# nii-yamagishilab/NELE-GAN

Measured on AMD Instinct MI355X. Metric: utterances/sec per GAN_epoch step (G+D+metric loss), higher is better.
Workload: dtype bf16

## Files before the change

### nele_gan_amd/csrc/haspi.hip

```cpp
#include "common.h"
#include "ws_arena.h"
#include <type_traits>
#include <cstdlib>

#define HP_NCH 32
#define HP_FS 24000.0
#define HP_LEVEL 65.0
#define HP_NBASIS 6
#define HP_NMOD 10
#define HP_NWIN 32769
#define HP_NTAB 512
#define HP_SPACE 9
#define HP_NFILT 52
#define HP_NHALF 26

typedef float hp_env_t;

struct HaspiWs {
    double* win;
    float* r24;
    double* mid;
    hp_env_t* ctl;
    hp_env_t* env;
    double* bw;
// ... 477 lines not shown
    if (loss < thrOHC) { attnOHC = 0.8 * loss; attnIHC = 0.2 * loss; }
    else { attnOHC = 0.8 * thrOHC; attnIHC = 0.2 * thrOHC + (loss - thrOHC); }
    const double r = attnOHC / 50.0;
    const double BW = 1.0 + r + 2.0 * (r * r * r * r * r * r);
    const double lowknee = attnOHC + 30.0, upamp = 30.0 + 70.0 / CR0;
    const double CR = (100.0 - lowknee) / (upamp + attnOHC - lowknee);
    double* p = ws.loss + (size_t)sig * 5 * HP_NCH + ch;
    p[0] = attnOHC; p[HP_NCH] = BW; p[2 * HP_NCH] = lowknee; p[3 * HP_NCH] = CR; p[4 * HP_NCH] = attnIHC;
}

__device__ __forceinline__ void hp_rotate(double& cold, double& sold, double cn, double sn);
__device__ __forceinline__ double hp_gammatone_wave(const double* __restrict__ xin, int n24, const GtCoef c, double cf, int part,
                                                    hp_env_t* __restrict__ out) {
    const double tpt = 2.0 * M_PI / HP_FS;
    const double cn = cos(tpt * cf), sn = sin(tpt * cf);
    double cold = 1.0, sold = 0.0;
    double r0 = 0, r1 = 0, r2 = 0, r3 = 0;
    double ss = 0.0;
    for (int n0 = 0; n0 < n24; n0 += HP_CH) {
        double xc[HP_CH];
#pragma unroll
        for (int u = 0; u < HP_CH; ++u) xc[u] = xin[n0 + u];
        double eo[HP_CH];
#pragma unroll
        for (int u = 0; u < HP_CH; ++u) {
            if (n0 + u > 0) hp_rotate(cold, sold, cn, sn);
            const double xr = xc[u] * (part ? sold : cold);
            const double yr = xr + r0;
            r0 = c.a1 * xr + c.a1 * yr + r1;
            r1 = c.a5 * xr + c.a2 * yr + r2;
            r2 = c.a3 * yr + r3;
            r3 = c.a4 * yr;
            const double yo = lane_xor32(yr);
            const double e2 = yr * yr + yo * yo;
            eo[u] = e2;
            ss += (n0 + u < n24) ? e2 : 0.0;
        }
        if (part == 0) {
#pragma unroll
            for (int u = 0; u < HP_CH; ++u) out[(size_t)(n0 + u) * HP_NCH] = (hp_env_t)eo[u];
        }
    }
    return ss;
}

#define GS_RC 16
#define GS_LC 1536
#define GS_MAXC 160
__device__ __forceinline__ void hp_rotate(double& cold, double& sold, double cn, double sn) {
    const double arg = fma(sold, sn, cold * cn);
    sold = fma(sold, cn, -(cold * sn));
    cold = arg;
}
__device__ __forceinline__ void hp_gt_step(const GtCoef& c, double x, double y, double& r0, double& r1, double& r2, double& r3) {
    r0 = fma(c.a1, x + y, r1);
    r1 = fma(c.a5, x, fma(c.a2, y, r2));
    r2 = fma(c.a3, y, r3);
    r3 = c.a4 * y;
}
__global__ __launch_bounds__(128) void haspi_pmat_kernel(HaspiWs ws, int lc, int signal, int sig0, int nsig) {
    const int ch = threadIdx.x & 31, k = threadIdx.x >> 5;
    const int row = signal ? hp_row(blockIdx.x, sig0, nsig) : 0;
    const double BW = signal ? ws.bw[(size_t)row * HP_NCH + ch] : hp_bw1(ch);
    const GtCoef c = hp_gt(BW, hp_cfreq(ch));
    double r0 = (k == 0), r1 = (k == 1), r2 = (k == 2), r3 = (k == 3);
    for (int n = 0; n < lc; ++n) {
        const double yr = r0;
        r0 = c.a1 * yr + r1;
        r1 = c.a2 * yr + r2;
        r2 = c.a3 * yr + r3;
        r3 = c.a4 * yr;
    }
    double* P = ws.pmat + ((size_t)(signal ? 1 + row : 0) * HP_NCH + ch) * 16;
    P[0 * 4 + k] = r0; P[1 * 4 + k] = r1; P[2 * 4 + k] = r2; P[3 * 4 + k] = r3;
}

template <bool SIGNAL>
__global__ __launch_bounds__(64) void haspi_bank_prefix_kernel(HaspiWs ws, int sig0, int nsig) {
    const int row = hp_row(blockIdx.x, sig0, nsig), lane = threadIdx.x, ch = lane & 31;
    const int n24 = hp_n24(ws, row >> 1);
    const int nch = ((n24 + GS_RC - 1) / GS_RC * GS_RC + ws.lc - 1) / ws.lc;
    const double* P = ws.pmat + ((size_t)(SIGNAL ? 1 + row : 0) * HP_NCH + ch) * 16;
    double Pm[16];
#pragma unroll
    for (int q = 0; q < 16; ++q) Pm[q] = P[q];
    double* est = ws.est + (size_t)row * ws.nchunk * 256 + lane;
    double r0 = 0, r1 = 0, r2 = 0, r3 = 0;
    constexpr int G = 8;
    for (int j0 = 0; j0 < nch; j0 += G) {
        double e[G][4];
#pragma unroll
        for (int g = 0; g < G; ++g) {
            const int j = min(j0 + g, nch - 1);
#pragma unroll
            for (int q = 0; q < 4; ++q) e[g][q] = est[(size_t)j * 256 + 64 * q];
        }
#pragma unroll
        for (int g = 0; g < G; ++g) {
            if (j0 + g < nch) {
                double* o = est + (size_t)(j0 + g) * 256;
                o[0] = r0; o[64] = r1; o[128] = r2; o[192] = r3;
                const double t0 = ((Pm[0] * r0 + Pm[1] * r1) + (Pm[2] * r2 + Pm[3] * r3)) + e[g][0];
                const double t1 = ((Pm[4] * r0 + Pm[5] * r1) + (Pm[6] * r2 + Pm[7] * r3)) + e[g][1];
                const double t2 = ((Pm[8] * r0 + Pm[9] * r1) + (Pm[10] * r2 + Pm[11] * r3)) + e[g][2];
                const double t3 = ((Pm[12] * r0 + Pm[13] * r1) + (Pm[14] * r2 + Pm[15] * r3)) + e[g][3];
                r0 = t0; r1 = t1; r2 = t2; r3 = t3;
            }
        }
    }
}

#define GL_N 2048
#define GL_W 256
#define GL_U 8
__device__ __forceinline__ float hp_log2f(float x) { return __builtin_amdgcn_logf(x); }
__device__ __forceinline__ float hp_exp2f(float x) { return __builtin_amdgcn_exp2f(x); }
struct IhcC { double R2, R12C1, R23C2, a11, a12, a21, a22, denom, R1inv, c10, c11, c12, c20, c21, c22; };
__device__ __forceinline__ IhcC hp_ihc_consts() {
    const double delta = 2.0;
    const double tau1 = 0.001 * 2, tau2 = 0.001 * 60;
    const double T = 1 / HP_FS;
    const double R1 = 1 / delta, R2 = 0.5 * (1 - R1), R3 = R2;
    const double C1 = tau1 * (R1 + R2) / (R1 * R2);
    const double C2 = tau2 / ((R1 + R2) * R3);
    IhcC k;
    k.a11 = R1 + R2 + R1 * R2 * (C1 / T); k.a12 = -R1; k.a21 = -R3; k.a22 = R2 + R3 + R2 * R3 * (C2 / T);
    k.denom = 1.0 / (k.a11 * k.a22 - k.a21 * k.a12);
    k.R1inv = 1.0 / R1; k.R12C1 = R1 * R2 * (C1 / T); k.R23C2 = R2 * R3 * (C2 / T); k.R2 = R2;
    k.c10 = k.denom * k.a22 * k.R2;  k.c11 = k.denom * k.a22 * k.R12C1;  k.c12 = -k.denom * k.a12 * k.R23C2;
    k.c20 = -k.denom * k.a21 * k.R2; k.c21 = -k.denom * k.a21 * k.R12C1; k.c22 = k.denom * k.a11 * k.R23C2;
    return k;
}
__device__ __forceinline__ void hp_ihc_step(const IhcC& k, double V0, double& V1, double& V2) {
    const double t1 = fma(k.c12, V2, fma(k.c11, V1, V0 * k.c10));
    const double t2 = fma(k.c22, V2, fma(k.c21, V1, V0 * k.c20));
    V1 = t1; V2 = t2;
}

template <bool SIGNAL, bool PASS2, bool BM = false, bool GAIN = false>
__global__ __launch_bounds__(64) void haspi_bank_scan_kernel(HaspiWs ws, int sig0) {
    const int b = blockIdx.z, sig = sig0 + blockIdx.y, lane = threadIdx.x, ch = lane & 31;
    const int chunk = 2 * blockIdx.x + (lane >> 5);
    const int row = 2 * b + sig, lc = ws.lc;
    const int n24 = hp_n24(ws, b);
    const int n0 = chunk * lc, n1 = min(n0 + lc, (n24 + GS_RC - 1) / GS_RC * GS_RC);
    if (n0 >= n1) return;
    const double cf = hp_cfreq(ch);
    const GtCoef c = hp_gt(SIGNAL ? ws.bw[(size_t)row * HP_NCH + ch] : hp_bw1(ch), cf);
    const double tpt = 2.0 * M_PI / HP_FS;
    const double cn = cos(tpt * cf), sn = sin(tpt * cf);
    double* est = ws.est + ((size_t)row * ws.nchunk + chunk) * 256 + ch;
    double r0 = 0, r1 = 0, r2 = 0, r3 = 0, i0 = 0, i1 = 0, i2 = 0, i3 = 0;
    if (PASS2) {
        r0 = est[0]; r1 = est[64]; r2 = est[128]; r3 = est[192];
        i0 = est[32]; i1 = est[96]; i2 = est[160]; i3 = est[224];
    }
    double cold, sold;
    {
        const double ang = tpt * cf * (double)(n0 - 1);
        cold = cos(ang);
        sold = -sin(ang);
    }
    const double* xin = ws.mid + (size_t)row * ws.n24p;
    hp_env_t* out = (SIGNAL ? ws.env : ws.ctl) + ((size_t)row * ws.n24p) * HP_NCH + ch;
    float* cph = BM ? ws.cphi + ((size_t)row * ws.n24p) * HP_NCH + ch : nullptr;
    double ss = 0.0;
    const hp_env_t* ctl = ws.ctl + (size_t)row * ws.n24p * HP_NCH + ch;
    const float TEN_LOG10_2 = 3.0102999566398120f, LOG2_10_OVER_20 = 0.16609640474436813f;
    float slope = 0.f, c_off = 0.f, s_off = 0.f;
    double gz = 0.0, V1 = 0.0, V2 = 0.0;
    const double gb0 = 0.095107983402496, ga1 = -0.809784033195007;
    const IhcC ik = hp_ihc_consts();
    float knee = 30.0f, attn = 0.f;
    if (GAIN) {
        const HpLoss ls = hp_loss(ws, sig, ch);
        slope = (float)(1.0 - (1.0 / ls.CR));
        knee = (float)ls.lowknee; attn = (float)ls.attnOHC;
        c_off = (float)(HP_LEVEL + 20.0 * log10(hp_gt(hp_bw1(ch), cf).gain));
        s_off = (float)(HP_LEVEL - ls.attnIHC + 20.0 * log10(c.gain));
        for (int n = max(0, n0 - GL_W); n < n0; n += GL_U) {
            float gc[GL_U];
#pragma unroll
            for (int u = 0; u < GL_U; ++u) gc[u] = ctl[(size_t)(n + u) * HP_NCH];
#pragma unroll
            for (int u = 0; u < GL_U; ++u) {
                float le = c_off + TEN_LOG10_2 * hp_log2f(gc[u]);
                le = fminf(fmaxf(le, knee), 100.0f);
                const double gx = (double)hp_exp2f((-attn - (le - knee) * slope) * LOG2_10_OVER_20);
                const double y = gb0 * gx + gz;
                gz = gb0 * gx - ga1 * y;
            }
        }
    }
    for (int nb = n0; nb < n1; nb += GS_RC) {
        double xc[GS_RC];
        const hp_env_t* ctl_nb = ctl + (size_t)nb * HP_NCH;
        hp_env_t* out_nb = out + (size_t)nb * HP_NCH;
        float* cph_nb = BM ? cph + (size_t)nb * HP_NCH : nullptr;
#pragma unroll
        for (int u = 0; u < GS_RC / 2; ++u) {
            const double2 v = *reinterpret_cast<const double2*>(xin + nb + 2 * u);
            xc[2 * u] = v.x; xc[2 * u + 1] = v.y;
        }
        float eo[GS_RC], co[BM ? GS_RC : 1];
        auto bank = [&](auto tail_tag) {
            constexpr bool TAIL = decltype(tail_tag)::value;
#pragma unroll
            for (int u = 0; u < GS_RC; ++u) {
                hp_rotate(cold, sold, cn, sn);
                const double xr = xc[u] * cold, xi = xc[u] * sold;
                const double yr = xr + r0, yi = xi + i0;
                hp_gt_step(c, xr, yr, r0, r1, r2, r3);
                hp_gt_step(c, xi, yi, i0, i1, i2, i3);
                if (PASS2) {
                    const double e2 = yr * yr + yi * yi;
                    eo[u] = (float)e2;
                    if (!SIGNAL || BM) ss += (!TAIL || nb + u < n24) ? e2 : 0.0;
                    if (BM) co[u] = e2 > 0.0 ? (float)((yr * cold + yi * sold) / sqrt(e2)) : 0.f;
                }
            }
        };
        if (PASS2 && (!SIGNAL || BM) && nb + GS_RC > n24) bank(std::true_type{}); else bank(std::false_type{});
        if (GAIN) {
            float gc[GS_RC];
#pragma unroll
            for (int u = 0; u < GS_RC; ++u) gc[u] = ctl_nb[u * HP_NCH];
#pragma unroll
            for (int u = 0; u < GS_RC; ++u) {
                float le = c_off + TEN_LOG10_2 * hp_log2f(gc[u]);
                le = fminf(fmaxf(le, knee), 100.0f);
                const double gx = (double)hp_exp2f((-attn - (le - knee) * slope) * LOG2_10_OVER_20);
                const double yl = gb0 * gx + gz;
                gz = gb0 * gx - ga1 * yl;
                const float g = (float)yl;
                float y = s_off + TEN_LOG10_2 * hp_log2f(g * g * eo[u]);
                y = y > 0.0f ? y : 0.0f;
                eo[u] = y;
                hp_ihc_step(ik, (double)y, V1, V2);
            }
        }
        if (PASS2) {
#pragma unroll
            for (int u = 0; u < GS_RC; ++u) out_nb[u * HP_NCH] = eo[u];
            if (BM) {
#pragma unroll
                for (int u = 0; u < GS_RC; ++u) cph_nb[u * HP_NCH] = co[u];
            }
        }
    }
    if (!PASS2) {
        est[0] = r0; est[64] = r1; est[128] = r2; est[192] = r3;
        est[32] = i0; est[96] = i1; est[160] = i2; est[224] = i3;
    } else if (!SIGNAL) {
        ws.ssp[((size_t)row * ws.nchunk + chunk) * HP_NCH + ch] = ss;
    } else if (BM) {
        ws.sse[((size_t)row * ws.nchunk + chunk) * HP_NCH + ch] = ss;
    }
    if (GAIN) {
        const int ncg = (ws.n24p + ws.lcg - 1) / ws.lcg;
        double* ihe = ws.ihe + ((size_t)row * ncg + chunk) * 64 + ch;
        ihe[0] = V1; ihe[32] = V2;
    }
}

template <bool SIGNAL>
__global__ __launch_bounds__(512) void haspi_bank_tail_kernel(HaspiWs ws, int sig0, int nsig, int full, int nrows) {
    __shared__ double stage[2][64][GS_RC + 1];
    __shared__ int wred[8];
    const int id = (int)blockIdx.x, slot = id >> 3, cgrp = slot & 3, rest = slot >> 2;
    const int ncg = (ws.nchunk + 63) / 64;
    const int ridx = (rest / ncg) * 8 + (id & 7);
    if (ridx >= nrows) return;
    const int row = hp_row(ridx, sig0, nsig), b = row >> 1;
    const int tid = threadIdx.x, lane = tid & 63, wv = tid >> 6, ch = 8 * cgrp + wv;
    const int c0 = 64 * (rest % ncg), chunk = c0 + lane, lc = ws.lc;
    const int n24 = hp_n24(ws, b), nend = (n24 + GS_RC - 1) / GS_RC * GS_RC;
    const int n0 = chunk * lc, n1 = min(n0 + lc, nend);
    const bool live = n0 < n1;
    const double cf = hp_cfreq(ch);
    const double BW = SIGNAL ? ws.bw[(size_t)row * HP_NCH + ch] : hp_bw1(ch);
    const GtCoef c = hp_gt(BW, cf);
    const double tpt = 2.0 * M_PI / HP_FS;
    int W;
    {
        const double la = BW * tpt * (24.7 + cf / 9.26449) * 1.019;
        const double npk = fmax(3.0 / la, 1.0);
        const double peak = 3.0 * log(npk) - la * npk;
        double nn = 60.0 / la;
        for (int it = 0; it < 6; ++it) nn = (50.66 - peak + 3.0 * log(nn)) / la;
        W = ((int)nn + 1 + GS_RC) / GS_RC * GS_RC;
        W = min(W, lc);
        if (full == 1) W = lc;
        if (full == 2) W = GS_RC;
    }
    if (lane == 0) wred[wv] = W;
    __syncthreads();
    int Wmax = wred[0];
#pragma unroll
    for (int q = 1; q < 8; ++q) Wmax = max(Wmax, wred[q]);
    const double cn = cos(tpt * cf), sn = sin(tpt * cf);
    double cold, sold;
    {
        const double ang = tpt * cf * (double)(n1 - W - 1);
        cold = cos(ang);
        sold = -sin(ang);
    }
    const double* xin = ws.mid + (size_t)row * ws.n24p;
    const int cc = tid >> 3, part = tid & 7;
    const int cn0 = (c0 + cc) * lc, cn1 = min(cn0 + lc, nend);
    const double* psrc = xin + (cn1 - Wmax + 2 * part);
    const int pfirst = (cn0 < cn1) ? cn0 - (cn1 - Wmax + 2 * part) : 0x7fffffff;
    double2 pv = (0 >= pfirst) ? *reinterpret_cast<const double2*>(psrc) : make_double2(0.0, 0.0);
    double r0 = 0, r1 = 0, r2 = 0, r3 = 0, i0 = 0, i1 = 0, i2 = 0, i3 = 0;
    const int tjoin = Wmax - W;
    for (int t = 0, it = 0; t < Wmax; t += GS_RC, ++it) {
        double (*st)[GS_RC + 1] = stage[it & 1];
        st[cc][2 * part] = pv.x; st[cc][2 * part + 1] = pv.y;
        __syncthreads();
        if (t + GS_RC < Wmax) pv = (t + GS_RC >= pfirst) ? *reinterpret_cast<const double2*>(psrc + t + GS_RC) : make_double2(0.0, 0.0);
        if (t >= tjoin) {
            double xc[GS_RC];
#pragma unroll
            for (int u = 0; u < GS_RC; ++u) xc[u] = st[lane][u];
#pragma unroll
            for (int u = 0; u < GS_RC; ++u) {
                hp_rotate(cold, sold, cn, sn);
                const double xr = xc[u] * cold, xi = xc[u] * sold;
                const double yr = xr + r0, yi = xi + i0;
                hp_gt_step(c, xr, yr, r0, r1, r2, r3);
                hp_gt_step(c, xi, yi, i0, i1, i2, i3);
            }
        }
    }
    if (live) {
        double* est = ws.est + ((size_t)row * ws.nchunk + chunk) * 256 + ch;
        est[0] = r0; est[64] = r1; est[128] = r2; est[192] = r3;
        est[32] = i0; est[96] = i1; est[160] = i2; est[224] = i3;
    }
}
__global__ void haspi_bw_kernel(HaspiWs ws, int sig0, int nsig) {
    const int row = hp_row(blockIdx.x, sig0, nsig), ch = threadIdx.x;
    const double bw1 = hp_bw1(ch);
    const GtCoef cc = hp_gt(bw1, hp_cfreq(ch));
    const int n24 = hp_n24(ws, row >> 1);
    const int nch = (n24 + ws.lc - 1) / ws.lc;
    double ss = 0.0;
    for (int c = 0; c < nch; ++c) ss += ws.ssp[((size_t)row * ws.nchunk + c) * HP_NCH + ch];
    ss *= cc.gain * cc.gain;
    const double cdB = 20.0 * log10(sqrt(ss / (double)n24)) + HP_LEVEL;
    const double bwmin = hp_loss(ws, row & 1, ch).BWmin;
    double BW;
    if (cdB < 50.0) BW = bwmin;
    else if (cdB > 100.0) BW = bw1;
    else BW = bwmin + ((cdB - 50.0) / 50.0) * (bw1 - bwmin);
    ws.bw[(size_t)row * HP_NCH + ch] = BW;
}

#ifdef NELE_AB
__global__ __launch_bounds__(64) void haspi_control_kernel(HaspiWs ws, int sig0) {
    const int b = blockIdx.y, sig = sig0 + blockIdx.x, lane = threadIdx.x, part = lane >> 5, ch = lane & 31;
    const double cf = hp_cfreq(ch), bw1 = hp_bw1(ch);
    const double* xin = ws.mid + ((size_t)b * 2 + sig) * ws.n24p;
    hp_env_t* out = ws.ctl + (((size_t)b * 2 + sig) * ws.n24p) * HP_NCH + ch;
    const GtCoef cc = hp_gt(bw1, cf);
    const int n24 = hp_n24(ws, b);
    const double ss = (cc.gain * cc.gain) * hp_gammatone_wave(xin, n24, cc, cf, part, out);
    if (part == 0) {
        const double cdB = 20.0 * log10(sqrt(ss / (double)n24)) + HP_LEVEL;
        const double bwmin = hp_loss(ws, sig, ch).BWmin;
        double BW;
        if (cdB < 50.0) BW = bwmin;
        else if (cdB > 100.0) BW = bw1;
        else BW = bwmin + ((cdB - 50.0) / 50.0) * (bw1 - bwmin);
        ws.bw[((size_t)b * 2 + sig) * HP_NCH + ch] = BW;
    }
}
#endif

#ifdef NELE_AB
__global__ __launch_bounds__(64) void haspi_signal_kernel(HaspiWs ws, int sig0) {
    const int b = blockIdx.y, sig = sig0 + blockIdx.x, lane = threadIdx.x, part = lane >> 5, ch = lane & 31;
    const double cf = hp_cfreq(ch);
    const double BW = ws.bw[((size_t)b * 2 + sig) * HP_NCH + ch];
// ... 26 lines not shown
    if (idx >= nrows) return;
    hp_env_t* g = ws.ctl + ((size_t)hp_row(idx, sig0, nsig) * ws.n24p) * HP_NCH + (lane & 31);
    const double b0 = 0.095107983402496, a1 = -0.809784033195007;
    double z = 0.0;
    for (int n0 = 0; n0 < ws.n24; n0 += HP_CH) {
        double gx[HP_CH];
#pragma unroll
        for (int u = 0; u < HP_CH; ++u) gx[u] = (double)g[(size_t)(n0 + u) * HP_NCH];
#pragma unroll
        for (int u = 0; u < HP_CH; ++u) {
            const double y = b0 * gx[u] + z;
            z = b0 * gx[u] - a1 * y;
            gx[u] = y;
        }
#pragma unroll
        for (int u = 0; u < HP_CH; ++u) g[(size_t)(n0 + u) * HP_NCH] = (hp_env_t)gx[u];
    }
}
#endif

#ifdef NELE_AB
__global__ void haspi_sl_kernel(HaspiWs ws, size_t per_row, int sig0, int nsig) {
    const int ch = (int)(threadIdx.x & 31), row = hp_row(blockIdx.y, sig0, nsig);
    const double sgain = hp_gt(ws.bw[(size_t)row * HP_NCH + ch], hp_cfreq(ch)).gain;
    const double attnIHC = hp_loss(ws, row & 1, ch).attnIHC;
    const size_t base = (size_t)row * per_row;
    for (size_t r = blockIdx.x * (size_t)blockDim.x + threadIdx.x; r < per_row; r += (size_t)gridDim.x * blockDim.x) {
        const size_t i = base + r;
        const double c = (double)ws.ctl[i] * (sgain * sqrt((double)ws.env[i]));
        const double y = HP_LEVEL - attnIHC + 20.0 * log10(c + 1.0e-30);
        ws.env[i] = (hp_env_t)(y < 0.0 ? 0.0 : y);
    }
}
#endif


__global__ __launch_bounds__(256) void haspi_gain_lp_sl_kernel(HaspiWs ws, int sig0, int nsig) {
    const int ch = threadIdx.x & 31, row = hp_row(blockIdx.y, sig0, nsig);
    const int n0 = (blockIdx.x * 8 + (threadIdx.x >> 5)) * ws.lcg;
    const int n24r = (hp_n24(ws, row >> 1) + HP_CH - 1) / HP_CH * HP_CH;
    if (n0 >= n24r) return;
    const int n1 = min(n0 + ws.lcg, n24r);
    const double cgain = hp_gt(hp_bw1(ch), hp_cfreq(ch)).gain;
    const double sgain = hp_gt(ws.bw[(size_t)row * HP_NCH + ch], hp_cfreq(ch)).gain;
    const HpLoss ls = hp_loss(ws, row & 1, ch);
    const float slope = (float)(1.0 - (1.0 / ls.CR)), knee = (float)ls.lowknee, attn = (float)ls.attnOHC;
    const float TEN_LOG10_2 = 3.0102999566398120f, LOG2_10_OVER_20 = 0.16609640474436813f;
    const float c_off = (float)(HP_LEVEL + 20.0 * log10(cgain)), s_off = (float)(HP_LEVEL - ls.attnIHC + 20.0 * log10(sgain));
    const double b0 = 0.095107983402496, a1 = -0.809784033195007;
    const hp_env_t* ctl = ws.ctl + (size_t)row * ws.n24p * HP_NCH + ch;
    hp_env_t* env = ws.env + (size_t)row * ws.n24p * HP_NCH + ch;
    double z = 0.0;
    const IhcC ik = hp_ihc_consts();
    double V1 = 0.0, V2 = 0.0;
    for (int n = max(0, n0 - GL_W); n < n1; n += GL_U) {
        float gc[GL_U], ev[GL_U];
        double gx[GL_U];
        const bool live = n >= n0;
#pragma unroll
        for (int u = 0; u < GL_U; ++u) gc[u] = ctl[(size_t)(n + u) * HP_NCH];
        if (live) {
#pragma unroll
            for (int u = 0; u < GL_U; ++u) ev[u] = env[(size_t)(n + u) * HP_NCH];
        }
#pragma unroll
        for (int u = 0; u < GL_U; ++u) {
            float le = c_off + TEN_LOG10_2 * hp_log2f(gc[u]);
            le = fminf(fmaxf(le, knee), 100.0f);
            gx[u] = (double)hp_exp2f((-attn - (le - knee) * slope) * LOG2_10_OVER_20);
        }
#pragma unroll
        for (int u = 0; u < GL_U; ++u) {
            const double y = b0 * gx[u] + z;
            z = b0 * gx[u] - a1 * y;
            gx[u] = y;
        }
        if (live) {
#pragma unroll
            for (int u = 0; u < GL_U; ++u) {
                const float g = (float)gx[u];
                float y = s_off + TEN_LOG10_2 * hp_log2f(g * g * ev[u]);
                y = y > 0.0f ? y : 0.0f;
                env[(size_t)(n + u) * HP_NCH] = y;
                hp_ihc_step(ik, (double)y, V1, V2);
            }
        }
    }
    const int ncg = (ws.n24p + ws.lcg - 1) / ws.lcg;
    double* ihe = ws.ihe + ((size_t)row * ncg + (n0 / ws.lcg)) * 64 + ch;
    ihe[0] = V1; ihe[32] = V2;
}

__global__ __launch_bounds__(32) void haspi_ihc_prefix_kernel(HaspiWs ws, int sig0, int nsig) {
    const int row = hp_row(blockIdx.x, sig0, nsig), ch = threadIdx.x;
    const int n24 = hp_n24(ws, row >> 1), ncg = (ws.n24p + ws.lcg - 1) / ws.lcg;
    const int nch = ((n24 + HP_CH - 1) / HP_CH * HP_CH + ws.lcg - 1) / ws.lcg;
    double* ihe = ws.ihe + ((size_t)row * ncg) * 64 + ch;
    const double p00 = ws.pihc[0], p01 = ws.pihc[1], p10 = ws.pihc[2], p11 = ws.pihc[3];
    double V1 = 0.0, V2 = 0.0;
    constexpr int G = 8;
    for (int j0 = 0; j0 < nch; j0 += G) {
        double e1[G], e2[G];
#pragma unroll
        for (int g = 0; g < G; ++g) { const int j = min(j0 + g, nch - 1); e1[g] = ihe[(size_t)j * 64]; e2[g] = ihe[(size_t)j * 64 + 32]; }
#pragma unroll
        for (int g = 0; g < G; ++g) {
            if (j0 + g < nch) {
                ihe[(size_t)(j0 + g) * 64] = V1; ihe[(size_t)(j0 + g) * 64 + 32] = V2;
                const double t1 = (p00 * V1 + p01 * V2) + e1[g], t2 = (p10 * V1 + p11 * V2) + e2[g];
                V1 = t1; V2 = t2;
            }
        }
    }
}

#define IF_L 51
#ifdef NELE_AB
__global__ __launch_bounds__(128) void haspi_ihc_fir_kernel(HaspiWs ws, int sig0, int nsig) {
    __shared__ float ring[64][128];
    const int tid = threadIdx.x, ch = tid & 31, row = hp_row(blockIdx.y, sig0, nsig), b = row >> 1;
    const int lcf = ws.lcg * ws.fmul;
    const int chunk = blockIdx.x * 4 + (tid >> 5), n0 = chunk * lcf;
    const int n24 = hp_n24(ws, b), nsub = hp_nsub(ws, b);
    const int ncg = (ws.n24p + ws.lcg - 1) / ws.lcg;
    const int last = (n24 - 1) / lcf;
#pragma unroll
    for (int q = 0; q < 64; ++q) ring[q][tid] = 0.f;
    if (chunk > last) return;
    const int sh = ws.shift[(size_t)b * HP_NCH + ch];
    const int n1 = (chunk == last) ? n24 + 9 + 26 : n0 + lcf;
    const IhcC k = hp_ihc_consts();
    const double* ihe = ws.ihe + ((size_t)row * ncg + (size_t)chunk * ws.fmul) * 64 + ch;
    double V1 = ihe[0], V2 = ihe[32];
    const hp_env_t* e = ws.env + ((size_t)row * ws.n24p) * HP_NCH + ch;
    int nstart = n0;
    if (chunk > 0) {
        nstart = n0 - IF_L;
        float hb[IF_L];
#pragma unroll
        for (int q = 0; q < IF_L; ++q) hb[q] = e[(size_t)(n0 - 1 - q) * HP_NCH];
        const double iR12 = 1.0 / k.R12C1, iR23 = 1.0 / k.R23C2;
#pragma unroll
        for (int q = 0; q < IF_L; ++q) {
            const double V0 = (double)hb[q];
            const double b1 = k.a11 * V1 + k.a12 * V2, b2 = k.a21 * V1 + k.a22 * V2;
            V1 = (b1 - V0 * k.R2) * iR12;
            V2 = b2 * iR23;
        }
    }
    double* lp = ws.lp + ((size_t)row * ws.nlp) * HP_NCH + ch;
    if (chunk == 0) {
        for (int i = 0; i < nsub && 9 * i + 26 - sh < 0; ++i) lp[(size_t)i * HP_NCH] = 0.0;
    }
    const double phi = 2.0 * M_PI / (double)IF_L, rc = cos(phi), rs = sin(phi);
    double s0 = 0.0, s1r = 0.0, s1i = 0.0;
    int icur, ph;
    {
        const int t = nstart + sh - 26;
        icur = (t >= 0) ? t / 9 : -((-t + 8) / 9);
        ph = t - 9 * icur;
    }
    float nx[GL_U];
#pragma unroll
    for (int u = 0; u < GL_U; ++u) nx[u] = e[(size_t)min(nstart + u, n24 - 1) * HP_NCH];
    for (int nb = nstart; nb < n1; nb += GL_U) {
        float ex[GL_U], olds[GL_U], news[GL_U];
#pragma unroll
        for (int u = 0; u < GL_U; ++u) ex[u] = nx[u];
#pragma unroll
        for (int u = 0; u < GL_U; ++u) nx[u] = e[(size_t)min(nb + GL_U + u, n24 - 1) * HP_NCH];
#pragma unroll
        for (int u = 0; u < GL_U; ++u) olds[u] = ring[(nb + u - IF_L) & 63][tid];
        double yv = 0.0;
        int yi = -1;
#pragma unroll
        for (int u = 0; u < GL_U; ++u) {
            const int n = nb + u;
            float o = 0.f;
            if (n + sh < n24) {
                const double V0 = (double)ex[u];
                hp_ihc_step(k, V0, V1, V2);
                const double out = (V0 - V1) * k.R1inv;
                o = (float)(out < 0.0 ? 0.0 : out);
            }
            news[u] = o;
            const double dx = (double)o - (double)olds[u];
            s0 += dx;
            { const double nr = (rc * s1r - rs * s1i) + dx; s1i = rc * s1i + rs * s1r; s1r = nr; }
            const bool due = (ph == 0) && n >= n0 && n < n1;
            yv = due ? (0.5 * s0 - 0.5 * s1r) * (1.0 / 25.5) : yv;
            yi = due ? icur : yi;
            const bool wrap = ph == 8;
            ph = wrap ? 0 : ph + 1;
            icur += wrap ? 1 : 0;
        }
#pragma unroll
        for (int u = 0; u < GL_U; ++u) ring[(nb + u) & 63][tid] = news[u];
        if (yi >= 0 && yi < nsub) lp[(size_t)yi * HP_NCH] = yv;
    }
}
#endif

#define IF_G 9
#define IF_SLOTS 6
__global__ __launch_bounds__(128) void haspi_ihc_fir9_kernel(HaspiWs ws, int sig0, int nsig) {
    const int tid = threadIdx.x, ch = tid & 31, row = hp_row(blockIdx.y, sig0, nsig), b = row >> 1;
    const int lcf = ws.lcg * ws.fmul;
    const int chunk = blockIdx.x * 4 + (tid >> 5), n0 = chunk * lcf;
    const int n24 = hp_n24(ws, b), nsub = hp_nsub(ws, b);
    const int ncg = (ws.n24p + ws.lcg - 1) / ws.lcg;
    const int last = (n24 - 1) / lcf;
    if (chunk > last) return;
    const int sh = ws.shift[(size_t)b * HP_NCH + ch];
    const int n1 = (chunk == last) ? n24 + 9 + 26 : n0 + lcf;
    const IhcC k = hp_ihc_consts();
    const double* ihe = ws.ihe + ((size_t)row * ncg + (size_t)chunk * ws.fmul) * 64 + ch;
    double V1 = ihe[0], V2 = ihe[32];
    const hp_env_t* e = ws.env + ((size_t)row * ws.n24p) * HP_NCH + ch;
    const int ul = (((26 - sh) % 9) + 9) % 9;
    int nG = (chunk > 0) ? (n0 - IF_L) / 9 * 9 : 0;
    if (chunk > 0) {
        const int cnt = n0 - nG;
        float hb[IF_L + IF_G - 1];
#pragma unroll
        for (int q = 0; q < IF_L + IF_G - 1; ++q) hb[q] = e[(size_t)(n0 - 1 - q) * HP_NCH];
        const double idet = 1.0 / (k.c11 * k.c22 - k.c12 * k.c21);
#pragma unroll
        for (int q = 0; q < IF_L + IF_G - 1; ++q) {
            const double V0 = (double)hb[q];
            const double w1 = V1 - k.c10 * V0, w2 = V2 - k.c20 * V0;
            const double o1 = (k.c22 * w1 - k.c12 * w2) * idet, o2 = (k.c11 * w2 - k.c21 * w1) * idet;
            V1 = q < cnt ? o1 : V1;
            V2 = q < cnt ? o2 : V2;
        }
    }
    double* lp = ws.lp + ((size_t)row * ws.nlp) * HP_NCH + ch;
    const double phi = 2.0 * M_PI / (double)IF_L, rc = cos(phi), rs = sin(phi);
    double s0 = 0.0, s1r = 0.0, s1i = 0.0;
    const hp_env_t* ep = e + (size_t)nG * HP_NCH;
    float nx[IF_G];
#pragma unroll
    for (int u = 0; u < IF_G; ++u) nx[u] = ep[u * HP_NCH];
    float dl[IF_SLOTS * IF_G];
#pragma unroll
    for (int q = 0; q < IF_SLOTS * IF_G; ++q) dl[q] = 0.f;
    int i = nG / 9;
    auto group = [&](auto slot_tag, auto edge_tag) {
        constexpr int S = decltype(slot_tag)::value, S1 = (S + 1) % IF_SLOTS;
        constexpr bool EDGE = decltype(edge_tag)::value;
        float ex[IF_G];
#pragma unroll
        for (int u = 0; u < IF_G; ++u) ex[u] = nx[u];
#pragma unroll
        for (int u = 0; u < IF_G; ++u) nx[u] = ep[(IF_G + u) * HP_NCH];
        double z = 0.0;
#pragma unroll
        for (int u = 0; u < IF_G; ++u) {
            const double V0 = (double)ex[u];
            hp_ihc_step(k, V0, V1, V2);
            float o = (float)fmax((V0 - V1) * k.R1inv, 0.0);
            if (EDGE) o = (nG + u + sh < n24) ? o : 0.f;
            const float old = (u < 6) ? dl[S * IF_G + u + 3] : dl[S1 * IF_G + u - 6];
            dl[S * IF_G + u] = o;
            const double dx = (double)o - (double)old;
            s0 += dx;
            { const double nr = fma(-rs, s1i, fma(rc, s1r, dx)); s1i = fma(rc, s1i, rs * s1r); s1r = nr; }
            z = (u == ul) ? s0 - s1r : z;
        }
        const int nE = nG + ul;
        if (nE >= n0 && nE < n1 && i < ws.nlp) lp[(size_t)i * HP_NCH] = (0.5 * z) * (1.0 / 25.5);
        nG += IF_G; ep += IF_G * HP_NCH; ++i;
    };
#define IF_GROUP(S)                                                                                              \
    if (nG >= n1) break;                                                                                         \
    if (nG + (IF_G - 1) + sh >= n24) group(std::integral_constant<int, S>{}, std::true_type{});                  \
    else group(std::integral_constant<int, S>{}, std::false_type{});
    for (;;) { IF_GROUP(0) IF_GROUP(1) IF_GROUP(2) IF_GROUP(3) IF_GROUP(4) IF_GROUP(5) }
#undef IF_GROUP
}

#ifdef NELE_AB
__global__ __launch_bounds__(64) void haspi_ihc_kernel(HaspiWs ws, int sig0, int nsig, int nrows) {
    const int lane = threadIdx.x, idx = 2 * blockIdx.x + (lane >> 5);
    if (idx >= nrows) return;
    const int row = hp_row(idx, sig0, nsig), n24 = hp_n24(ws, row >> 1);
    hp_env_t* e = ws.env + ((size_t)row * ws.n24p) * HP_NCH + (lane & 31);
    const IhcC k = hp_ihc_consts();
    double V1 = 0.0, V2 = 0.0;
    for (int n0 = 0; n0 < n24; n0 += HP_CH) {
        double ex[HP_CH];
#pragma unroll
        for (int u = 0; u < HP_CH; ++u) ex[u] = (double)e[(size_t)(n0 + u) * HP_NCH];
#pragma unroll
        for (int u = 0; u < HP_CH; ++u) {
            const double V0 = ex[u];
            hp_ihc_step(k, V0, V1, V2);
            const double out = (V0 - V1) * k.R1inv;
            ex[u] = out < 0.0 ? 0.0 : out;
        }
#pragma unroll
        for (int u = 0; u < HP_CH; ++u) e[(size_t)(n0 + u) * HP_NCH] = (hp_env_t)ex[u];
    }
}
#endif

__global__ __launch_bounds__(64) void haspi_shift_kernel(HaspiWs ws) {
    const int b = blockIdx.x, ch = threadIdx.x;
    double gd = 0.0;
    if (ch < HP_NCH) {
        const GtCoef c = hp_gt(ws.bw[(size_t)b * 2 * HP_NCH + ch], hp_cfreq(ch));
        const double a = 0.25 * c.a1;
        gd = rint((c.a1 + 2.0 * c.a5) / (1.0 + c.a1 + c.a5) + 4.0 * a / (1.0 - a));
    }
    double mn = (ch < HP_NCH) ? gd : 1e300, mx = (ch < HP_NCH) ? gd : -1e300;
    for (int o = 32; o > 0; o >>= 1) { mn = fmin(mn, __shfl_xor(mn, o, 64)); mx = fmax(mx, __shfl_xor(mx, o, 64)); }
    if (ch < HP_NCH) ws.shift[(size_t)b * HP_NCH + ch] = (int)((mx - mn) - (gd - mn));
    if (b == 0 && ch < 2) {
        const IhcC k = hp_ihc_consts();
        double V1 = (ch == 0), V2 = (ch == 1);
        for (int n = 0; n < ws.lcg; ++n) hp_ihc_step(k, 0.0, V1, V2);
        ws.pihc[ch] = V1; ws.pihc[2 + ch] = V2;
    }
    if (b == 0 && ch < HP_NFILT) ws.benv[ch] = (0.5 - 0.5 * cospi(2.0 * (double)ch / 51.0)) / 25.5;
    if (b == 0) {
        const int nfirs[10] = {614, 614, 614, 384, 244, 152, 96, 60, 38, 24};
        for (int k = 0; k < 10; ++k)
            for (int i = ch; i <= nfirs[k]; i += 64) ws.bkt[k * 616 + i] = (0.5 - 0.5 * cospi(2.0 * (double)i / (double)nfirs[k])) / (0.5 * (double)nfirs[k]);
    }
}

#define EF_SUB 16
#define EF_SPAN (EF_SUB * HP_SPACE + HP_NFILT)
#ifdef NELE_AB
__global__ __launch_bounds__(256) void haspi_envfilt_kernel(HaspiWs ws, int sig0) {
    __shared__ double xs[EF_SPAN][HP_NCH + 1];
    const int b = blockIdx.y, sig = sig0 + blockIdx.z, tid = threadIdx.x, ch = tid & 31;
    const int i0 = blockIdx.x * EF_SUB;
    const int n24 = hp_n24(ws, b), nsub = hp_nsub(ws, b);
    if (i0 >= nsub) return;
    const double* __restrict__ benv = ws.benv;
    const int s = ws.shift[(size_t)b * HP_NCH + ch];
    const hp_env_t* e = ws.env + (((size_t)b * 2 + sig) * ws.n24p) * HP_NCH + ch;
    const int mbase = HP_SPACE * i0 + HP_NHALF - (HP_NFILT - 1);
    {
        constexpr int NQ = (EF_SPAN + 7) / 8;
        double val[NQ];
#pragma unroll
        for (int u = 0; u < NQ; ++u) {
            const int q = (tid >> 5) + 8 * u;
            const int src = mbase + q - s;
            val[u] = (double)e[(size_t)min(max(src, 0), n24 - 1) * HP_NCH];
        }
#pragma unroll
        for (int u = 0; u < NQ; ++u) {
            const int q = (tid >> 5) + 8 * u;
            const int m = mbase + q, src = m - s;
            if (q < EF_SPAN) xs[q][ch] = (m >= 0 && m < n24 && src >= 0) ? val[u] : 0.0;
        }
    }
    __syncthreads();
    for (int li = tid >> 5; li < EF_SUB; li += 8) {
        const int i = i0 + li;
        if (i >= nsub) break;
        double acc = 0.0;
#pragma unroll 4
        for (int k = 0; k < HP_NFILT; ++k) acc += benv[k] * xs[HP_SPACE * li + (HP_NFILT - 1) - k][ch];
        ws.lp[(((size_t)b * 2 + sig) * ws.nlp + i) * HP_NCH + ch] = acc;
    }
}
#endif

#define CP_F 128
__device__ __forceinline__ void hp_stage_lp(const HaspiWs& ws, int b, const double* __restrict__ lp, int i0, int nsub, double (*tile)[HP_NCH + 1]) {
    const int nfr = min(CP_F, nsub - i0);
// ... 749 lines not shown
```

### nele_gan_amd/csrc/haspi_quality.h

```cpp
#define HQ_NWIN 384
#define HQ_NHALF 192
#define HQ_MAXLAG 24
#define HQ_NOUT 12
#define HQ_MAXBINS 2048

struct QualWs {
    double* sm;
    double* cov;
    double* msx;
    double* msy;
    double* corr;
    double* segl;
    int* qinfo;
    int nseg;
    unsigned long long seed;
    int noise;
    const long long* ids;
};

__device__ __forceinline__ int hq_nseg(int n24) { return 1 + n24 / HQ_NWIN + (n24 - HQ_NHALF) / HQ_NWIN; }
__device__ __forceinline__ double hq_win(int k) { return 0.5 - 0.5 * cospi(2.0 * (double)k / (double)(HQ_NWIN - 1)); }

__device__ __forceinline__ unsigned long long hq_mix(unsigned long long z) {
    z += 0x9E3779B97F4A7C15ull;
    z = (z ^ (z >> 30)) * 0xBF58476D1CE4E5B9ull;
    z = (z ^ (z >> 27)) * 0x94D049BB133111EBull;
    return z ^ (z >> 31);
}
__device__ __forceinline__ float hq_gauss(unsigned long long seed, unsigned long long idx) {
    const unsigned long long r = hq_mix(seed ^ hq_mix(idx));
    const float u1 = ((float)(unsigned)(r >> 40) + 1.0f) * (1.0f / 16777216.0f);
    const float u2 = (float)(unsigned)((r >> 8) & 0xFFFFFFu) * (1.0f / 16777216.0f);
    return sqrtf(-2.0f * __logf(u1)) * __cosf(6.283185307179586f * u2);
}

__global__ __launch_bounds__(256) void hq_ihc_bm_kernel(HaspiWs ws, QualWs q, int sig0, int nsig) {
    const int tid = threadIdx.x, ch = tid & 31, row = hp_row(blockIdx.y, sig0, nsig);
    const int chunk = blockIdx.x * 8 + (tid >> 5), n0 = chunk * ws.lcg;
    const int n24 = hp_n24(ws, row >> 1);
    if (n0 >= n24) return;
    const int n1 = min(n0 + ws.lcg, (n24 + GL_U - 1) / GL_U * GL_U);
    const int ncg = (ws.n24p + ws.lcg - 1) / ws.lcg;
    const IhcC k = hp_ihc_consts();
    const double* ihe = ws.ihe + ((size_t)row * ncg + chunk) * 64 + ch;
    double V1 = ihe[0], V2 = ihe[32];
    hp_env_t* e = ws.env + ((size_t)row * ws.n24p) * HP_NCH + ch;
    float* c = ws.cphi + ((size_t)row * ws.n24p) * HP_NCH + ch;
    const float gn = q.noise ? 1.7782794100389227e-4f : 0.f;
    unsigned long long base = ((unsigned long long)row * HP_NCH + ch) * (unsigned long long)ws.n24p, key = q.seed;
    if (q.noise == 2) {
        key = hq_mix(q.seed ^ hq_mix((unsigned long long)q.ids[row >> 1]));
        base = (unsigned long long)((row & 1) * HP_NCH + ch) << 32;
    }
    for (int nb = n0; nb < n1; nb += GL_U) {
        float ev[GL_U], cv[GL_U];
#pragma unroll
        for (int u = 0; u < GL_U; ++u) { ev[u] = e[(size_t)(nb + u) * HP_NCH]; cv[u] = c[(size_t)(nb + u) * HP_NCH]; }
#pragma unroll
        for (int u = 0; u < GL_U; ++u) {
            const double V0 = (double)ev[u];
            hp_ihc_step(k, V0, V1, V2);
            double out = (V0 - V1) * k.R1inv;
            out = out < 0.0 ? 0.0 : out;
            ev[u] = (float)out;
            float bm = (float)((out + 1.0e-30) * (double)cv[u]);
            if (q.noise) bm += gn * hq_gauss(key, base + (unsigned long long)(nb + u));
            cv[u] = bm;
        }
#pragma unroll
        for (int u = 0; u < GL_U; ++u) { e[(size_t)(nb + u) * HP_NCH] = ev[u]; c[(size_t)(nb + u) * HP_NCH] = cv[u]; }
    }
}

__device__ __forceinline__ void hq_segment(int seg, int nseg, int& st, int& len, int& woff) {
    st = seg * HQ_NHALF;
    if (seg == 0) { len = HQ_NHALF; woff = HQ_NHALF; }
    else if (seg == nseg - 1) { len = HQ_NHALF; woff = 0; }
    else { len = HQ_NWIN; woff = 0; }
}

__global__ void hq_corr_kernel(QualWs q) {
    const int t = threadIdx.x, half = t >> 6, i = t & 63;
    if (i > 2 * HQ_MAXLAG) return;
    const int l = i - HQ_MAXLAG, N = half ? HQ_NHALF : HQ_NWIN, off = half ? HQ_NHALF : 0;
    double s = 0.0;
    for (int n = 0; n < N; ++n) {
        const int m = n + l;
        if (m >= 0 && m < N) s += hq_win(off + m) * hq_win(off + n);
    }
    q.corr[half * 64 + i] = 1.0 / s;
}

#define HQ_XR (HQ_NWIN + 2 * HQ_MAXLAG + 4)
#define HQ_TROWS 640
template <int MODE>
__global__ __launch_bounds__(128) void hq_segment_kernel(HaspiWs ws, QualWs q) {
    __shared__ __attribute__((aligned(16))) float tile[HQ_TROWS][8];
    __shared__ float xs[HQ_XR][8];
    __shared__ float ys[HQ_NWIN][8];
    __shared__ double wtab[HQ_NWIN];
    __shared__ double part[16][8][2];
    __shared__ double mx[16][8];
    const int tid = threadIdx.x, c = tid & 7, k16 = tid >> 3, b = blockIdx.z, ch0 = blockIdx.y * 8, ch = ch0 + c;
    const int n24 = hp_n24(ws, b), nseg = hq_nseg(n24), seg = blockIdx.x;
    if (seg >= nseg) return;
    int st, N, woff;
    hq_segment(seg, nseg, st, N, woff);
    for (int k = tid; k < N; k += 128) wtab[k] = hq_win(woff + k);
    const int sh = ws.shift[(size_t)b * HP_NCH + ch];
    int smin = sh, smax = sh;
#pragma unroll
    for (int o = 1; o < 8; o <<= 1) { smin = min(smin, __shfl_xor(smin, o, 64)); smax = max(smax, __shfl_xor(smax, o, 64)); }
    const int base = st - smax;
    const int rows = min(N + smax - smin, HQ_TROWS);
    const int roff = smax - sh;
// ... 495 lines not shown
```

Measured before the change: 7438.

## Diagonalize IHC adaptation recurrence and use Chebyshev recurrence for carrier rotation

After: 7514 (median of 6 runs). Within noise of the previous version (+1.0%).

```diff
diff --git a/nele_gan_amd/csrc/haspi.hip b/nele_gan_amd/csrc/haspi.hip
--- a/nele_gan_amd/csrc/haspi.hip
+++ b/nele_gan_amd/csrc/haspi.hip
@@ -553,6 +553,11 @@
     sold = fma(sold, cn, -(cold * sn));
     cold = arg;
 }
+__device__ __forceinline__ void hp_rotate3(double& cold, double& cprev, double& sold, double& sprev, double k2) {
+    const double cnew = fma(k2, cold, -cprev), snew = fma(k2, sold, -sprev);
+    cprev = cold; sprev = sold;
+    cold = cnew; sold = snew;
+}
 __device__ __forceinline__ void hp_gt_step(const GtCoef& c, double x, double y, double& r0, double& r1, double& r2, double& r3) {
     r0 = fma(c.a1, x + y, r1);
     r1 = fma(c.a5, x, fma(c.a2, y, r2));
@@ -616,7 +621,7 @@
 #define GL_U 8
 __device__ __forceinline__ float hp_log2f(float x) { return __builtin_amdgcn_logf(x); }
 __device__ __forceinline__ float hp_exp2f(float x) { return __builtin_amdgcn_exp2f(x); }
-struct IhcC { double R2, R12C1, R23C2, a11, a12, a21, a22, denom, R1inv, c10, c11, c12, c20, c21, c22; };
+struct IhcC { double l1, l2, il1, il2, g1, g2, R1inv; };
 __device__ __forceinline__ IhcC hp_ihc_consts() {
     const double delta = 2.0;
     const double tau1 = 0.001 * 2, tau2 = 0.001 * 60;
@@ -624,18 +629,32 @@
     const double R1 = 1 / delta, R2 = 0.5 * (1 - R1), R3 = R2;
     const double C1 = tau1 * (R1 + R2) / (R1 * R2);
     const double C2 = tau2 / ((R1 + R2) * R3);
+    const double a11 = R1 + R2 + R1 * R2 * (C1 / T), a12 = -R1, a21 = -R3, a22 = R2 + R3 + R2 * R3 * (C2 / T);
+    const double denom = 1.0 / (a11 * a22 - a21 * a12);
+    const double R12C1 = R1 * R2 * (C1 / T), R23C2 = R2 * R3 * (C2 / T);
+    const double c10 = denom * a22 * R2, c11 = denom * a22 * R12C1, c12 = -denom * a12 * R23C2;
+    const double c20 = -denom * a21 * R2, c21 = -denom * a21 * R12C1, c22 = denom * a11 * R23C2;
     IhcC k;
-    k.a11 = R1 + R2 + R1 * R2 * (C1 / T); k.a12 = -R1; k.a21 = -R3; k.a22 = R2 + R3 + R2 * R3 * (C2 / T);
-    k.denom = 1.0 / (k.a11 * k.a22 - k.a21 * k.a12);
-    k.R1inv = 1.0 / R1; k.R12C1 = R1 * R2 * (C1 / T); k.R23C2 = R2 * R3 * (C2 / T); k.R2 = R2;
-    k.c10 = k.denom * k.a22 * k.R2;  k.c11 = k.denom * k.a22 * k.R12C1;  k.c12 = -k.denom * k.a12 * k.R23C2;
-    k.c20 = -k.denom * k.a21 * k.R2; k.c21 = -k.denom * k.a21 * k.R12C1; k.c22 = k.denom * k.a11 * k.R23C2;
+    const double disc = sqrt((c11 - c22) * (c11 - c22) + 4.0 * c12 * c21);
+    k.l1 = 0.5 * ((c11 + c22) - disc); k.l2 = 0.5 * ((c11 + c22) + disc);
+    k.il1 = 1.0 / k.l1; k.il2 = 1.0 / k.l2;
+    const double u1x = k.l1 - c22, u1y = c21, u2x = c12, u2y = k.l2 - c11;
+    const double idet = 1.0 / (u1x * u2y - u2x * u1y);
+    const double beta1 = (u2y * c10 - u2x * c20) * idet, beta2 = (u1x * c20 - u1y * c10) * idet;
+    k.R1inv = 1.0 / R1;
+    k.g1 = (u1x * beta1) * k.R1inv; k.g2 = (u2x * beta2) * k.R1inv;
     return k;
 }
-__device__ __forceinline__ void hp_ihc_step(const IhcC& k, double V0, double& V1, double& V2) {
-    const double t1 = fma(k.c12, V2, fma(k.c11, V1, V0 * k.c10));
-    const double t2 = fma(k.c22, V2, fma(k.c21, V1, V0 * k.c20));
-    V1 = t1; V2 = t2;
+__device__ __forceinline__ void hp_ihc_state(const IhcC& k, double V0, double& z1, double& z2) {
+    z1 = fma(k.l1, z1, V0);
+    z2 = fma(k.l2, z2, V0);
+}
+__device__ __forceinline__ double hp_ihc_out(const IhcC& k, double V0, double z1, double z2) {
+    return fma(-k.g1, z1, fma(-k.g2, z2, V0 * k.R1inv));
+}
+__device__ __forceinline__ void hp_ihc_back(const IhcC& k, double V0, double& z1, double& z2) {
+    z1 = (z1 - V0) * k.il1;
+    z2 = (z2 - V0) * k.il2;
 }
 
 template <bool SIGNAL, bool PASS2, bool BM = false, bool GAIN = false>
@@ -669,7 +688,7 @@
     const hp_env_t* ctl = ws.ctl + (size_t)row * ws.n24p * HP_NCH + ch;
     const float TEN_LOG10_2 = 3.0102999566398120f, LOG2_10_OVER_20 = 0.16609640474436813f;
     float slope = 0.f, c_off = 0.f, s_off = 0.f;
-    double gz = 0.0, V1 = 0.0, V2 = 0.0;
+    double gz = 0.0, z1 = 0.0, z2 = 0.0;
     const double gb0 = 0.095107983402496, ga1 = -0.809784033195007;
     const IhcC ik = hp_ihc_consts();
     float knee = 30.0f, attn = 0.f;
@@ -737,7 +756,7 @@
                 float y = s_off + TEN_LOG10_2 * hp_log2f(g * g * eo[u]);
                 y = y > 0.0f ? y : 0.0f;
                 eo[u] = y;
-                hp_ihc_step(ik, (double)y, V1, V2);
+                hp_ihc_state(ik, (double)y, z1, z2);
             }
         }
         if (PASS2) {
@@ -760,7 +779,7 @@
     if (GAIN) {
         const int ncg = (ws.n24p + ws.lcg - 1) / ws.lcg;
         double* ihe = ws.ihe + ((size_t)row * ncg + chunk) * 64 + ch;
-        ihe[0] = V1; ihe[32] = V2;
+        ihe[0] = z1; ihe[32] = z2;
     }
 }
 
@@ -799,12 +818,12 @@
     int Wmax = wred[0];
 #pragma unroll
     for (int q = 1; q < 8; ++q) Wmax = max(Wmax, wred[q]);
-    const double cn = cos(tpt * cf), sn = sin(tpt * cf);
-    double cold, sold;
+    const double k2 = 2.0 * cos(tpt * cf);
+    double cold, sold, cprev, sprev;
     {
-        const double ang = tpt * cf * (double)(n1 - W - 1);
-        cold = cos(ang);
-        sold = -sin(ang);
+        const double ang = tpt * cf * (double)(n1 - W - 1), ang2 = tpt * cf * (double)(n1 - W - 2);
+        cold = cos(ang); sold = -sin(ang);
+        cprev = cos(ang2); sprev = -sin(ang2);
     }
     const double* xin = ws.mid + (size_t)row * ws.n24p;
     const int cc = tid >> 3, part = tid & 7;
@@ -820,16 +839,19 @@
         __syncthreads();
         if (t + GS_RC < Wmax) pv = (t + GS_RC >= pfirst) ? *reinterpret_cast<const double2*>(psrc + t + GS_RC) : make_double2(0.0, 0.0);
         if (t >= tjoin) {
-            double xc[GS_RC];
-#pragma unroll
-            for (int u = 0; u < GS_RC; ++u) xc[u] = st[lane][u];
-#pragma unroll
-            for (int u = 0; u < GS_RC; ++u) {
-                hp_rotate(cold, sold, cn, sn);
-                const double xr = xc[u] * cold, xi = xc[u] * sold;
-                const double yr = xr + r0, yi = xi + i0;
-                hp_gt_step(c, xr, yr, r0, r1, r2, r3);
-                hp_gt_step(c, xi, yi, i0, i1, i2, i3);
+#pragma unroll
+            for (int h = 0; h < GS_RC; h += GS_RC / 2) {
+                double xc[GS_RC / 2];
+#pragma unroll
+                for (int u = 0; u < GS_RC / 2; ++u) xc[u] = st[lane][h + u];
+#pragma unroll
+                for (int u = 0; u < GS_RC / 2; ++u) {
+                    hp_rotate3(cold, cprev, sold, sprev, k2);
+                    const double xr = xc[u] * cold, xi = xc[u] * sold;
+                    const double yr = xr + r0, yi = xi + i0;
+                    hp_gt_step(c, xr, yr, r0, r1, r2, r3);
+                    hp_gt_step(c, xi, yi, i0, i1, i2, i3);
+                }
             }
         }
     }
@@ -962,7 +984,7 @@
     hp_env_t* env = ws.env + (size_t)row * ws.n24p * HP_NCH + ch;
     double z = 0.0;
     const IhcC ik = hp_ihc_consts();
-    double V1 = 0.0, V2 = 0.0;
+    double z1 = 0.0, z2 = 0.0;
     for (int n = max(0, n0 - GL_W); n < n1; n += GL_U) {
         float gc[GL_U], ev[GL_U];
         double gx[GL_U];
@@ -992,13 +1014,13 @@
                 float y = s_off + TEN_LOG10_2 * hp_log2f(g * g * ev[u]);
                 y = y > 0.0f ? y : 0.0f;
                 env[(size_t)(n + u) * HP_NCH] = y;
-                hp_ihc_step(ik, (double)y, V1, V2);
+                hp_ihc_state(ik, (double)y, z1, z2);
             }
         }
     }
     const int ncg = (ws.n24p + ws.lcg - 1) / ws.lcg;
     double* ihe = ws.ihe + ((size_t)row * ncg + (n0 / ws.lcg)) * 64 + ch;
-    ihe[0] = V1; ihe[32] = V2;
+    ihe[0] = z1; ihe[32] = z2;
 }
 
 __global__ __launch_bounds__(32) void haspi_ihc_prefix_kernel(HaspiWs ws, int sig0, int nsig) {
@@ -1006,8 +1028,8 @@
     const int n24 = hp_n24(ws, row >> 1), ncg = (ws.n24p + ws.lcg - 1) / ws.lcg;
     const int nch = ((n24 + HP_CH - 1) / HP_CH * HP_CH + ws.lcg - 1) / ws.lcg;
     double* ihe = ws.ihe + ((size_t)row * ncg) * 64 + ch;
-    const double p00 = ws.pihc[0], p01 = ws.pihc[1], p10 = ws.pihc[2], p11 = ws.pihc[3];
-    double V1 = 0.0, V2 = 0.0;
+    const double p1 = ws.pihc[0], p2 = ws.pihc[1];
+    double z1 = 0.0, z2 = 0.0;
     constexpr int G = 8;
     for (int j0 = 0; j0 < nch; j0 += G) {
         double e1[G], e2[G];
@@ -1016,9 +1038,8 @@
 #pragma unroll
         for (int g = 0; g < G; ++g) {
             if (j0 + g < nch) {
-                ihe[(size_t)(j0 + g) * 64] = V1; ihe[(size_t)(j0 + g) * 64 + 32] = V2;
-                const double t1 = (p00 * V1 + p01 * V2) + e1[g], t2 = (p10 * V1 + p11 * V2) + e2[g];
-                V1 = t1; V2 = t2;
+                ihe[(size_t)(j0 + g) * 64] = z1; ihe[(size_t)(j0 + g) * 64 + 32] = z2;
+                z1 = fma(p1, z1, e1[g]); z2 = fma(p2, z2, e2[g]);
             }
         }
     }
@@ -1041,7 +1062,7 @@
     const int n1 = (chunk == last) ? n24 + 9 + 26 : n0 + lcf;
     const IhcC k = hp_ihc_consts();
     const double* ihe = ws.ihe + ((size_t)row * ncg + (size_t)chunk * ws.fmul) * 64 + ch;
-    double V1 = ihe[0], V2 = ihe[32];
+    double z1 = ihe[0], z2 = ihe[32];
     const hp_env_t* e = ws.env + ((size_t)row * ws.n24p) * HP_NCH + ch;
     int nstart = n0;
     if (chunk > 0) {
@@ -1049,14 +1070,8 @@
         float hb[IF_L];
 #pragma unroll
         for (int q = 0; q < IF_L; ++q) hb[q] = e[(size_t)(n0 - 1 - q) * HP_NCH];
-        const double iR12 = 1.0 / k.R12C1, iR23 = 1.0 / k.R23C2;
-#pragma unroll
-        for (int q = 0; q < IF_L; ++q) {
-            const double V0 = (double)hb[q];
-            const double b1 = k.a11 * V1 + k.a12 * V2, b2 = k.a21 * V1 + k.a22 * V2;
-            V1 = (b1 - V0 * k.R2) * iR12;
-            V2 = b2 * iR23;
-        }
+#pragma unroll
+        for (int q = 0; q < IF_L; ++q) hp_ihc_back(k, (double)hb[q], z1, z2);
     }
     double* lp = ws.lp + ((size_t)row * ws.nlp) * HP_NCH + ch;
     if (chunk == 0) {
@@ -1089,8 +1104,8 @@
             float o = 0.f;
             if (n + sh < n24) {
                 const double V0 = (double)ex[u];
-                hp_ihc_step(k, V0, V1, V2);
-                const double out = (V0 - V1) * k.R1inv;
+                hp_ihc_state(k, V0, z1, z2);
+                const double out = hp_ihc_out(k, V0, z1, z2);
                 o = (float)(out < 0.0 ? 0.0 : out);
             }
             news[u] = o;
@@ -1125,7 +1140,7 @@
     const int n1 = (chunk == last) ? n24 + 9 + 26 : n0 + lcf;
     const IhcC k = hp_ihc_consts();
     const double* ihe = ws.ihe + ((size_t)row * ncg + (size_t)chunk * ws.fmul) * 64 + ch;
-    double V1 = ihe[0], V2 = ihe[32];
+    double z1 = ihe[0], z2 = ihe[32];
     const hp_env_t* e = ws.env + ((size_t)row * ws.n24p) * HP_NCH + ch;
     const int ul = (((26 - sh) % 9) + 9) % 9;
     int nG = (chunk > 0) ? (n0 - IF_L) / 9 * 9 : 0;
@@ -1134,14 +1149,12 @@
         float hb[IF_L + IF_G - 1];
 #pragma unroll
         for (int q = 0; q < IF_L + IF_G - 1; ++q) hb[q] = e[(size_t)(n0 - 1 - q) * HP_NCH];
-        const double idet = 1.0 / (k.c11 * k.c22 - k.c12 * k.c21);
 #pragma unroll
         for (int q = 0; q < IF_L + IF_G - 1; ++q) {
-            const double V0 = (double)hb[q];
-            const double w1 = V1 - k.c10 * V0, w2 = V2 - k.c20 * V0;
-            const double o1 = (k.c22 * w1 - k.c12 * w2) * idet, o2 = (k.c11 * w2 - k.c21 * w1) * idet;
-            V1 = q < cnt ? o1 : V1;
-            V2 = q < cnt ? o2 : V2;
+            double o1 = z1, o2 = z2;
+            hp_ihc_back(k, (double)hb[q], o1, o2);
+            z1 = q < cnt ? o1 : z1;
+            z2 = q < cnt ? o2 : z2;
         }
     }
     double* lp = ws.lp + ((size_t)row * ws.nlp) * HP_NCH + ch;
@@ -1167,8 +1180,8 @@
 #pragma unroll
         for (int u = 0; u < IF_G; ++u) {
             const double V0 = (double)ex[u];
-            hp_ihc_step(k, V0, V1, V2);
-            float o = (float)fmax((V0 - V1) * k.R1inv, 0.0);
+            hp_ihc_state(k, V0, z1, z2);
+            float o = (float)fmax(hp_ihc_out(k, V0, z1, z2), 0.0);
             if (EDGE) o = (nG + u + sh < n24) ? o : 0.f;
             const float old = (u < 6) ? dl[S * IF_G + u + 3] : dl[S1 * IF_G + u - 6];
             dl[S * IF_G + u] = o;
@@ -1196,7 +1209,7 @@
     const int row = hp_row(idx, sig0, nsig), n24 = hp_n24(ws, row >> 1);
     hp_env_t* e = ws.env + ((size_t)row * ws.n24p) * HP_NCH + (lane & 31);
     const IhcC k = hp_ihc_consts();
-    double V1 = 0.0, V2 = 0.0;
+    double z1 = 0.0, z2 = 0.0;
     for (int n0 = 0; n0 < n24; n0 += HP_CH) {
         double ex[HP_CH];
 #pragma unroll
@@ -1204,8 +1217,8 @@
 #pragma unroll
         for (int u = 0; u < HP_CH; ++u) {
             const double V0 = ex[u];
-            hp_ihc_step(k, V0, V1, V2);
-            const double out = (V0 - V1) * k.R1inv;
+            hp_ihc_state(k, V0, z1, z2);
+            const double out = hp_ihc_out(k, V0, z1, z2);
             ex[u] = out < 0.0 ? 0.0 : out;
         }
 #pragma unroll
@@ -1225,11 +1238,11 @@
     double mn = (ch < HP_NCH) ? gd : 1e300, mx = (ch < HP_NCH) ? gd : -1e300;
     for (int o = 32; o > 0; o >>= 1) { mn = fmin(mn, __shfl_xor(mn, o, 64)); mx = fmax(mx, __shfl_xor(mx, o, 64)); }
     if (ch < HP_NCH) ws.shift[(size_t)b * HP_NCH + ch] = (int)((mx - mn) - (gd - mn));
-    if (b == 0 && ch < 2) {
+    if (b == 0 && ch == 0) {
         const IhcC k = hp_ihc_consts();
-        double V1 = (ch == 0), V2 = (ch == 1);
-        for (int n = 0; n < ws.lcg; ++n) hp_ihc_step(k, 0.0, V1, V2);
-        ws.pihc[ch] = V1; ws.pihc[2 + ch] = V2;
+        double z1 = 1.0, z2 = 1.0;
+        for (int n = 0; n < ws.lcg; ++n) hp_ihc_state(k, 0.0, z1, z2);
+        ws.pihc[0] = z1; ws.pihc[1] = z2; ws.pihc[2] = 0.0; ws.pihc[3] = 0.0;
     }
     if (b == 0 && ch < HP_NFILT) ws.benv[ch] = (0.5 - 0.5 * cospi(2.0 * (double)ch / 51.0)) / 25.5;
     if (b == 0) {
diff --git a/nele_gan_amd/csrc/haspi_quality.h b/nele_gan_amd/csrc/haspi_quality.h
--- a/nele_gan_amd/csrc/haspi_quality.h
+++ b/nele_gan_amd/csrc/haspi_quality.h
@@ -43,7 +43,7 @@
     const int ncg = (ws.n24p + ws.lcg - 1) / ws.lcg;
     const IhcC k = hp_ihc_consts();
     const double* ihe = ws.ihe + ((size_t)row * ncg + chunk) * 64 + ch;
-    double V1 = ihe[0], V2 = ihe[32];
+    double z1 = ihe[0], z2 = ihe[32];
     hp_env_t* e = ws.env + ((size_t)row * ws.n24p) * HP_NCH + ch;
     float* c = ws.cphi + ((size_t)row * ws.n24p) * HP_NCH + ch;
     const float gn = q.noise ? 1.7782794100389227e-4f : 0.f;
@@ -59,8 +59,8 @@
 #pragma unroll
         for (int u = 0; u < GL_U; ++u) {
             const double V0 = (double)ev[u];
-            hp_ihc_step(k, V0, V1, V2);
-            double out = (V0 - V1) * k.R1inv;
+            hp_ihc_state(k, V0, z1, z2);
+            double out = hp_ihc_out(k, V0, z1, z2);
             out = out < 0.0 ? 0.0 : out;
             ev[u] = (float)out;
             float bm = (float)((out + 1.0e-30) * (double)cv[u]);
```
